# TencentARC/SEED-Story

Hardware: AMD Instinct MI355X
Metric: story-steps/sec (text + 1024x1024 image) (higher is better)
Workload: dtype bf16

## Files before the change

seed-story_amd/csrc/ss_attn.hip:

```cpp
#include "ss_common.h"

namespace ss {

struct AttnArgs {
    const void *q, *k, *v;
    void* out;
    int q_len, kv_len, hd, n_heads;
    int64_t q_sb, q_sh, q_ss, k_sb, k_sh, k_ss, v_sb, v_sh, v_ss, o_sb, o_sh, o_ss;
    float scale;
    int causal_br;
    int xcd_heads;
    int ragged;
    int kv_len_b[8];
};

template <typename T> struct AttnMma;
template <> struct AttnMma<bf16_t> {
    static __device__ __forceinline__ f32x4_t run(const uint4& a, const uint4& b, f32x4_t c) {
        return __builtin_amdgcn_mfma_f32_16x16x32_bf16(__builtin_bit_cast(bf16x8_t, a),
                                                       __builtin_bit_cast(bf16x8_t, b), c, 0, 0, 0);
    }
};
template <> struct AttnMma<f16_t> {
    static __device__ __forceinline__ f32x4_t run(const uint4& a, const uint4& b, f32x4_t c) {
// ... 896 lines not shown

#if SS_EXPERIMENTAL
template <typename T>
__global__ __launch_bounds__(256) __attribute__((amdgpu_waves_per_eu(2)))
void cross_attn64_kernel(const AttnArgs a, int n_items, int items_per_block, int chunks_per_pair) {
    constexpr int HD = 64, NDB = 4, NKB = 4, NKS = 2;
    const int tid = threadIdx.x, lane = tid & 63;
    const int wid = __builtin_amdgcn_readfirstlane(tid >> 6);
    const int l15 = lane & 15, grp = lane >> 4;
    const float sl2 = a.scale * 1.4426950408889634f;
    const uint4 ones = make_uint4(OnesFrag<T>::kPair, OnesFrag<T>::kPair, OnesFrag<T>::kPair, OnesFrag<T>::kPair);
    const int kvl = a.kv_len;
    const bool o_vec = ((a.o_ss | a.o_sh | a.o_sb) & 3) == 0;
    int it = blockIdx.x * items_per_block;
    int it_end = it + items_per_block;
    if (it_end > n_items) it_end = n_items;
    if (it >= it_end) return;

    uint4 kf[NKB][NKS];
    uint4 vf[NKB / 2][NDB];
    int cur_pair = -1;
    auto load_q = [&](int item, uint4 (&qf)[2][NKS]) {
        const int pair = item / chunks_per_pair, chunk = item - pair * chunks_per_pair;
        const int b = pair / a.n_heads, h = pair - b * a.n_heads;
        const T* __restrict__ qp = (const T*)a.q + (int64_t)b * a.q_sb + (int64_t)h * a.q_sh;
#pragma unroll
        for (int qb = 0; qb < 2; ++qb) {
            const int qi = chunk * 128 + wid * 32 + qb * 16 + l15;
#pragma unroll
            for (int ks = 0; ks < NKS; ++ks)
                qf[qb][ks] = qi < a.q_len ? ld16(qp + (int64_t)qi * a.q_ss + ks * 32 + grp * 8) : make_uint4(0, 0, 0, 0);
        }
    };
    uint4 qf[2][NKS], qn[2][NKS];
    load_q(it, qf);
    for (; it < it_end; ++it) {
        const bool more = it + 1 < it_end;
        if (more) load_q(it + 1, qn);
        const int pair = it / chunks_per_pair, chunk = it - pair * chunks_per_pair;
        const int b = pair / a.n_heads, h = pair - b * a.n_heads;
        if (pair != cur_pair) {
            cur_pair = pair;
            const T* __restrict__ kp = (const T*)a.k + (int64_t)b * a.k_sb + (int64_t)h * a.k_sh;
            const T* __restrict__ vp = (const T*)a.v + (int64_t)b * a.v_sb + (int64_t)h * a.v_sh;
#pragma unroll
            for (int kb = 0; kb < NKB; ++kb) {
                const int key = kb * 16 + l15;
#pragma unroll
                for (int ks = 0; ks < NKS; ++ks)
                    kf[kb][ks] = key < kvl ? ld16(kp + (int64_t)key * a.k_ss + ks * 32 + grp * 8) : make_uint4(0, 0, 0, 0);
            }
#pragma unroll
            for (int kp2 = 0; kp2 < NKB / 2; ++kp2)
#pragma unroll
                for (int db = 0; db < NDB; ++db) {
                    uint32_t w[4];
#pragma unroll
                    for (int j = 0; j < 8; j += 2) {
                        const int k0 = (2 * kp2 + (j >> 2)) * 16 + grp * 4 + (j & 3), k1 = k0 + 1;
                        const uint32_t lo = k0 < kvl ? (uint32_t)(vp + (int64_t)k0 * a.v_ss + db * 16 + l15)->v : 0u;
                        const uint32_t hi = k1 < kvl ? (uint32_t)(vp + (int64_t)k1 * a.v_ss + db * 16 + l15)->v : 0u;
                        w[j >> 1] = lo | (hi << 16);
                    }
                    vf[kp2][db] = make_uint4(w[0], w[1], w[2], w[3]);
                }
        }
        f32x4_t s[2][NKB];
#pragma unroll
        for (int kb = 0; kb < NKB; ++kb) {
            s[0][kb] = f32x4_t{0.f, 0.f, 0.f, 0.f};
            s[1][kb] = f32x4_t{0.f, 0.f, 0.f, 0.f};
#pragma unroll
            for (int ks = 0; ks < NKS; ++ks) {
                s[0][kb] = AttnMma<T>::run(kf[kb][ks], qf[0][ks], s[0][kb]);
                s[1][kb] = AttnMma<T>::run(kf[kb][ks], qf[1][ks], s[1][kb]);
            }
        }
        uint4 pfrag[2][NKB / 2];
#pragma unroll
        for (int qb = 0; qb < 2; ++qb) {
            if (kvl < 64) {
#pragma unroll
                for (int kb = 0; kb < NKB; ++kb)
#pragma unroll
                    for (int r = 0; r < 4; ++r)
                        if (kb * 16 + grp * 4 + r >= kvl) s[qb][kb][r] = -1e30f;
            }
            float tmax = -1e30f;
#pragma unroll
            for (int kb = 0; kb < NKB; ++kb)
#pragma unroll
                for (int r = 0; r < 4; ++r) tmax = fmaxf(tmax, s[qb][kb][r]);
            tmax = fmaxf(tmax, __shfl_xor(tmax, 16, 64));
            tmax = fmaxf(tmax, __shfl_xor(tmax, 32, 64));
            const float nm = -fmaxf(tmax, -1e29f) * sl2;
#pragma unroll
            for (int kp2 = 0; kp2 < NKB / 2; ++kp2) {
                float pf[8];
#pragma unroll
                for (int r = 0; r < 4; ++r) {
                    pf[r] = __builtin_amdgcn_exp2f(fmaf(s[qb][2 * kp2][r], sl2, nm));
                    pf[4 + r] = __builtin_amdgcn_exp2f(fmaf(s[qb][2 * kp2 + 1][r], sl2, nm));
                }
                pfrag[qb][kp2] = pack<T>(pf);
            }
        }
        f32x4_t o[2][NDB], osum[2];
#pragma unroll
        for (int qb = 0; qb < 2; ++qb) {
            osum[qb] = f32x4_t{0.f, 0.f, 0.f, 0.f};
#pragma unroll
            for (int i = 0; i < NDB; ++i) o[qb][i] = f32x4_t{0.f, 0.f, 0.f, 0.f};
        }
#pragma unroll
        for (int kp2 = 0; kp2 < NKB / 2; ++kp2) {
            osum[0] = AttnMma<T>::run(ones, pfrag[0][kp2], osum[0]);
            osum[1] = AttnMma<T>::run(ones, pfrag[1][kp2], osum[1]);
#pragma unroll
            for (int db = 0; db < NDB; ++db) {
                o[0][db] = AttnMma<T>::run(vf[kp2][db], pfrag[0][kp2], o[0][db]);
                o[1][db] = AttnMma<T>::run(vf[kp2][db], pfrag[1][kp2], o[1][db]);
            }
        }
#pragma unroll
        for (int qb = 0; qb < 2; ++qb) {
            const int qi = chunk * 128 + wid * 32 + qb * 16 + l15;
            if (qi >= a.q_len) continue;
            const float l = osum[qb][0];
            const float inv = l > 0.f ? 1.0f / l : 0.f;
            T* op = (T*)a.out + (int64_t)b * a.o_sb + (int64_t)h * a.o_sh + (int64_t)qi * a.o_ss;
#pragma unroll
            for (int db = 0; db < NDB; ++db) {
                const int d = db * 16 + grp * 4;
                if (o_vec) {
                    float pk[8] = {o[qb][db][0] * inv, o[qb][db][1] * inv, o[qb][db][2] * inv, o[qb][db][3] * inv, 0, 0, 0, 0};
                    const uint4 u = pack<T>(pk);
                    *reinterpret_cast<uint2*>(op + d) = make_uint2(u.x, u.y);
                } else {
#pragma unroll
                    for (int r = 0; r < 4; ++r) Tr<T>::st(op + d + r, o[qb][db][r] * inv);
                }
            }
        }
        if (more) {
#pragma unroll
            for (int qb = 0; qb < 2; ++qb)
#pragma unroll
                for (int ks = 0; ks < NKS; ++ks) qf[qb][ks] = qn[qb][ks];
        }
    }
}

template <typename T>
static int cross_attn64_launch(const AttnArgs& a, int64_t batch, hipStream_t s) {
    const int cpp = cdiv(a.q_len, 128);
    const int64_t n_items = batch * a.n_heads * cpp;
    static int n_cu = 0;
    if (n_cu == 0) {
        int dev = 0;
        hipDeviceProp_t p;
        if (hipGetDevice(&dev) == hipSuccess && hipGetDeviceProperties(&p, dev) == hipSuccess) n_cu = p.multiProcessorCount;
        if (n_cu <= 0) n_cu = 256;
    }
    const int64_t max_blocks = (int64_t)2 * n_cu;
    const int ipb = (int)((n_items + max_blocks - 1) / max_blocks);
    const int grid = (int)((n_items + ipb - 1) / ipb);
    hipLaunchKernelGGL((cross_attn64_kernel<T>), dim3((unsigned)grid), dim3(256), 0, s, a, (int)n_items, ipb, cpp);
    SS_LAUNCH_CHECK("cross_attn64");
    return SS_OK;
}

#endif

template <typename T, bool PIPE>
static int flash3p_launch(const AttnArgs& a, int64_t batch, hipStream_t s) {
    const int64_t kv_tiles = a.ragged ? 3 : cdiv(a.kv_len, kBKV);
    const size_t lds = (size_t)(kv_tiles < 3 && !PIPE ? (kv_tiles < 1 ? 1 : kv_tiles) : 3) * 2 * kBKV * 64 * 2;
    const int64_t bh = batch * a.n_heads;
    const int aw = knob(K_attn_waves);
    const bool many = a.ragged || a.kv_len >= 512;
    const bool w16 = !PIPE && (aw == 16 || (aw == 0 && many && a.q_len >= 2048 && (int64_t)cdiv(a.q_len, 512) * bh >= 1024));
    const bool w8 = !PIPE && !w16 && (aw == 8 || (aw == 0 && many && a.q_len >= 512 && (int64_t)cdiv(a.q_len, 256) * bh >= 1024));
    const int nqb = cdiv(a.q_len, w16 ? 512 : w8 ? 256 : 128);
    AttnArgs a2 = a;
    dim3 grid((unsigned)nqb, (unsigned)bh);
    a2.xcd_heads = 0;
    if (bh % 8 == 0 && nqb > 1 && knob(K_attn_xcd)) {
        a2.xcd_heads = nqb;
        grid = dim3((unsigned)(nqb * bh), 1);
    }
    if constexpr (!PIPE) {
        if (w16) {
            hipLaunchKernelGGL((flash_attn3p_kernel<T, 64, false, 16>), grid, dim3(1024), lds, s, a2);
            SS_LAUNCH_CHECK("flash_attn3p");
            return SS_OK;
        }
        if (w8) {
            hipLaunchKernelGGL((flash_attn3p_kernel<T, 64, false, 8>), grid, dim3(512), lds, s, a2);
            SS_LAUNCH_CHECK("flash_attn3p");
            return SS_OK;
        }
    }
    hipLaunchKernelGGL((flash_attn3p_kernel<T, 64, PIPE>), grid, dim3(256), lds, s, a2);
    SS_LAUNCH_CHECK("flash_attn3p");
    return SS_OK;
}

template <typename T, int HD, bool VSWZ>
static int flash3_launch_hd(const AttnArgs& a, int64_t batch, hipStream_t s) {
    const size_t lds = (size_t)(HD <= 64 ? 3 : 2) * 2 * kBKV * HD * 2;
    const int nqb = cdiv(a.q_len, 128);
    const int64_t bh = batch * a.n_heads;
    AttnArgs a2 = a;
    dim3 grid((unsigned)nqb, (unsigned)bh);
    a2.xcd_heads = 0;
    if (bh % 8 == 0 && nqb > 1 && knob(K_attn_xcd)) {
        a2.xcd_heads = nqb;
        grid = dim3((unsigned)(nqb * bh), 1);
    }
    hipLaunchKernelGGL((flash_attn3_kernel<T, HD, VSWZ>), grid, dim3(256), lds, s, a2);
    SS_LAUNCH_CHECK("flash_attn3");
    return SS_OK;
}

#if SS_EXPERIMENTAL
template <typename T, int HD>
static int flash2_launch_hd(const AttnArgs& a, int64_t batch, hipStream_t s) {
    const size_t lds = (size_t)(HD <= 64 ? 3 : 2) * 2 * kBKV * HD * 2;
    dim3 grid((unsigned)cdiv(a.q_len, 128), (unsigned)(batch * a.n_heads));
    hipLaunchKernelGGL((flash_attn2_kernel<T, HD>), grid, dim3(256), lds, s, a);
    SS_LAUNCH_CHECK("flash_attn2");
    return SS_OK;
}
#endif

template <typename T, int HD>
static int flash_launch_hd(const AttnArgs& a, int64_t batch, hipStream_t s) {
    constexpr int V = Tr<T>::kVec;
    const size_t lds = ((size_t)kBKV * (HD + V) + (size_t)HD * (kBKV + V)) * sizeof(T);
    dim3 grid((unsigned)cdiv(a.q_len, kBQ), (unsigned)(batch * a.n_heads));
    hipLaunchKernelGGL((flash_attn_kernel<T, HD>), grid, dim3(256), lds, s, a);
    SS_LAUNCH_CHECK("flash_attn");
    return SS_OK;
}

template <typename T>
int attention_launch(const AttnArgs& a, int64_t batch, hipStream_t s) {
    constexpr int V = Tr<T>::kVec;
    SS_REQUIRE(a.hd % V == 0 && a.hd > 0 && a.hd <= 128, "attention: head_dim %d unsupported", a.hd);
    SS_REQUIRE(a.q_ss % V == 0 && a.k_ss % V == 0 && a.v_ss % V == 0 && a.q_sh % V == 0 && a.k_sh % V == 0 &&
                   a.v_sh % V == 0 && a.q_sb % V == 0 && a.k_sb % V == 0 && a.v_sb % V == 0,
               "attention: strides must be multiples of %d elements", V);
    SS_REQUIRE(!a.causal_br || a.kv_len >= a.q_len, "attention: causal needs kv_len >= q_len");
    if (a.q_len == 0 || batch == 0) return SS_OK;
    SS_REQUIRE(a.kv_len > 0, "attention: kv_len == 0");
    if constexpr (V == 8) {
        const int ver = knob(K_attn_ver);
#if SS_EXPERIMENTAL
        if (a.hd == 64 && a.kv_len <= 64 && !a.causal_br && !a.ragged && a.q_len >= 128 && ver >= 3 && knob(K_attn_cross64))
            return cross_attn64_launch<T>(a, batch, s);
#endif
        if (ver == 5 && a.q_len >= 32 && a.hd <= 64) return flash3p_launch<T, true>(a, batch, s);
        if (ver == 6 && a.q_len >= 32 && a.hd <= 64) return flash3p_launch<T, false>(a, batch, s);
        if (ver >= 3 && a.q_len >= 32) {
            if (ver == 3 || ver >= 5) {
                if (a.hd <= 64) return flash3_launch_hd<T, 64, true>(a, batch, s);
                return flash3_launch_hd<T, 128, true>(a, batch, s);
            }
            if (a.hd <= 64) return flash3_launch_hd<T, 64, false>(a, batch, s);
            return flash3_launch_hd<T, 128, false>(a, batch, s);
        }
#if SS_EXPERIMENTAL
        if (ver == 2 && a.q_len >= 32) {
            if (a.hd <= 64) return flash2_launch_hd<T, 64>(a, batch, s);
            return flash2_launch_hd<T, 128>(a, batch, s);
        }
#else
        SS_REQUIRE(ver != 2, "attention: attn_ver 2 (flash v2) is only in the EXPERIMENTAL=1 build");
#endif
    }
    if (a.hd <= 64) return flash_launch_hd<T, 64>(a, batch, s);
    return flash_launch_hd<T, 128>(a, batch, s);
}

int attention_dev(const AttnArgs& a, int64_t batch, int dtype, hipStream_t s) {
    return SS_DISPATCH(dtype, attention_launch, a, batch, s);
}

template <typename T>
__device__ __forceinline__ uint4 rope_pack(const T* row_h, const T* cos_t, const T* sin_t, int pos, int hd, int d0) {
    constexpr int V = Tr<T>::kVec;
    const int half = hd >> 1;
    float x[V], xp[V], c[V], sn[V], o[V];
    unpack<T>(ld16(row_h + d0), x);
    unpack<T>(ld16(row_h + (d0 < half ? d0 + half : d0 - half)), xp);
    unpack<T>(ld16(cos_t + (int64_t)pos * hd + d0), c);
    unpack<T>(ld16(sin_t + (int64_t)pos * hd + d0), sn);
    const float sign = d0 < half ? -1.f : 1.f;
#pragma unroll
    for (int j = 0; j < V; ++j) o[j] = Tr<T>::rnd(Tr<T>::rnd(x[j] * c[j]) + Tr<T>::rnd(sign * xp[j] * sn[j]));
    return pack<T>(o);
}

struct DecodeArgs {
    const void* q;
    const void* qkv_raw;
    void *kc, *vc;
    const void *cos_t, *sin_t;
    float* part;
    const int32_t* kv_len_dev;
    const int32_t* pos_dev;
    const int32_t* done_flag;
    int hd, n_heads, cap, nsplit;
    float scale;
    int nb, state_stride;
    int64_t q_stride, cache_stride, part_stride, out_stride;
};

template <typename T>
__global__ __launch_bounds__(256) void attn_decode_kernel(const DecodeArgs a0) {
    DecodeArgs a = a0;
    {
        const int b = blockIdx.z;
        const int64_t so = (int64_t)b * a.state_stride;
        if (a.done_flag) a.done_flag += so;
        a.kv_len_dev += so;
        if (a.pos_dev) a.pos_dev += so;
        if (a.q) a.q = (const T*)a.q + b * a.q_stride;
        if (a.qkv_raw) a.qkv_raw = (const T*)a.qkv_raw + b * a.q_stride;
        a.kc = (T*)a.kc + b * a.cache_stride;
        a.vc = (T*)a.vc + b * a.cache_stride;
        a.part += b * a.part_stride;
    }
    constexpr int V = Tr<T>::kVec;
    constexpr int KPT = 4;
    extern __shared__ __attribute__((aligned(16))) char smem_raw[];
    float* sm = reinterpret_cast<float*>(smem_raw);
    if (a.done_flag && *a.done_flag) return;
    const int h = blockIdx.x, sp = blockIdx.y, tid = threadIdx.x;
    const int hd = a.hd;
    const int LPK = hd / V, NKG = 256 / LPK;
    const int kg = tid / LPK, dl = tid % LPK, d0 = dl * V;
    const bool fused = a.qkv_raw != nullptr;
    const int n_old = *a.kv_len_dev;
    const int kv_len = n_old + (fused ? 1 : 0);
    const int chunk = (kv_len + a.nsplit - 1) / a.nsplit;
    const int k_lo = sp * chunk;
    const int k_hi = min(kv_len, k_lo + chunk);
    const T* kh = (const T*)a.kc + (int64_t)h * a.cap * hd;
    const T* vh = (const T*)a.vc + (int64_t)h * a.cap * hd;
    const int E = a.n_heads * hd;

    auto load_kv = [&](int base, uint4 (&kk)[KPT], uint4 (&vv)[KPT]) {
#pragma unroll
        for (int i = 0; i < KPT; ++i) {
            const int key = base + i * NKG;
            if (key < k_hi && !(fused && key == n_old)) {
                kk[i] = ld16(kh + (int64_t)key * hd + d0);
                vv[i] = ld16(vh + (int64_t)key * hd + d0);
            } else {
                kk[i] = make_uint4(0, 0, 0, 0);
                vv[i] = make_uint4(0, 0, 0, 0);
            }
        }
    };
    uint4 kk[KPT], vv[KPT];
    int base = k_lo + kg;
    if (base < k_hi) load_kv(base, kk, vv);

    uint4 qv, knew = make_uint4(0, 0, 0, 0), vnew = make_uint4(0, 0, 0, 0);
    if (fused) {
        const T* raw = (const T*)a.qkv_raw;
        const int pos = *a.pos_dev;
        qv = rope_pack<T>(raw + (int64_t)h * hd, (const T*)a.cos_t, (const T*)a.sin_t, pos, hd, d0);
        if (n_old >= k_lo && n_old < k_hi) {
            knew = rope_pack<T>(raw + E + (int64_t)h * hd, (const T*)a.cos_t, (const T*)a.sin_t, pos, hd, d0);
            vnew = ld16(raw + 2 * E + (int64_t)h * hd + d0);
            if (kg == (n_old - k_lo) % NKG && n_old < a.cap) {
                st16((T*)a.kc + ((int64_t)h * a.cap + n_old) * hd + d0, knew);
                st16((T*)a.vc + ((int64_t)h * a.cap + n_old) * hd + d0, vnew);
            }
        }
    } else {
        qv = ld16((const T*)a.q + (int64_t)h * hd + d0);
    }

    float m = -1e30f, l = 0.f, acc[V];
#pragma unroll
    for (int j = 0; j < V; ++j) acc[j] = 0.f;
    while (base < k_hi) {
#pragma unroll
        for (int i = 0; i < KPT; ++i) {
            const int key = base + i * NKG;
            const bool is_new = fused && key == n_old;
            const uint4 kx = is_new ? knew : kk[i];
            const uint4 vx = is_new ? vnew : vv[i];
            float s = dot_pack<T>(kx, qv, 0.f);
            for (int o = LPK >> 1; o > 0; o >>= 1) s += __shfl_xor(s, o, 64);
            if (key < k_hi) {
                s *= a.scale;
                const float mn = fmaxf(m, s);
                const float al = expf(m - mn), p = expf(s - mn);
                float vf[V];
                unpack<T>(vx, vf);
                l = l * al + p;
#pragma unroll
                for (int j = 0; j < V; ++j) acc[j] = fmaf(p, vf[j], acc[j] * al);
                m = mn;
            }
        }
        base += NKG * KPT;
        if (base < k_hi) load_kv(base, kk, vv);
    }
    float* mine = sm + kg * (hd + 2);
    if (dl == 0) { mine[0] = m; mine[1] = l; }
#pragma unroll
    for (int j = 0; j < V; ++j) mine[2 + d0 + j] = acc[j];
    __syncthreads();
    float* rec = a.part + ((int64_t)h * a.nsplit + sp) * (hd + 2);
    if (tid < hd) {
        float mm = -1e30f;
        for (int g = 0; g < NKG; ++g) mm = fmaxf(mm, sm[g * (hd + 2)]);
        float lt = 0.f, ot = 0.f;
        for (int g = 0; g < NKG; ++g) {
            const float* r = sm + g * (hd + 2);
            const float w = r[1] > 0.f ? expf(r[0] - mm) : 0.f;
            lt = fmaf(w, r[1], lt);
            ot = fmaf(w, r[2 + tid], ot);
        }
        rec[2 + tid] = ot;
        if (tid == 0) { rec[0] = mm; rec[1] = lt; }
    }
}

template <typename T, int NS>
__global__ void attn_combine_kernel(const float* __restrict__ part, T* __restrict__ out,
                                    const int32_t* __restrict__ done_flag, int hd, int state_stride,
                                    int64_t part_stride, int64_t out_stride) {
    const int b = blockIdx.y;
    if (done_flag && done_flag[(int64_t)b * state_stride]) return;
    part += b * part_stride;
    out += b * out_stride;
    const int h = blockIdx.x, d = threadIdx.x;
    const float* rec = part + (int64_t)h * NS * (hd + 2);
    float ms[NS], ls[NS], os[NS];
#pragma unroll
    for (int s = 0; s < NS; ++s) {
        ms[s] = rec[s * (hd + 2)];
        ls[s] = rec[s * (hd + 2) + 1];
        os[s] = rec[s * (hd + 2) + 2 + d];
    }
    float m = -1e30f;
#pragma unroll
    for (int s = 0; s < NS; ++s) m = fmaxf(m, ms[s]);
    float l = 0.f, o = 0.f;
#pragma unroll
    for (int s = 0; s < NS; ++s) {
        const float w = ls[s] > 0.f ? expf(ms[s] - m) : 0.f;
        l = fmaf(w, ls[s], l);
        o = fmaf(w, os[s], o);
    }
    Tr<T>::st(out + (int64_t)h * hd + d, o / l);
}

static inline int decode_nsplit(int nb) {
    int n = knob(K_attn_decode_nsplit);
    if (n <= 0) n = 16 / (nb < 1 ? 1 : nb);
    return n <= 4 ? 4 : n <= 8 ? 8 : n <= 16 ? 16 : 32;
}

template <typename T>
int attn_decode_launch(const DecodeArgs& a0, void* out, int64_t n_heads, int64_t hd, hipStream_t s) {
    constexpr int V = Tr<T>::kVec;
    SS_REQUIRE(hd % V == 0 && 256 % (hd / V) == 0 && 64 % (hd / V) == 0 && hd <= 256,
               "attn_decode: head_dim %lld unsupported", (long long)hd);
    DecodeArgs a = a0;
    a.nsplit = decode_nsplit(a.nb);
    a.scale = 1.0f / sqrtf((float)hd);
    const int NKG = 256 / (int)(hd / V);
    const size_t lds = (size_t)NKG * (hd + 2) * sizeof(float);
    if (a.nb < 1) a.nb = 1;
    hipLaunchKernelGGL(attn_decode_kernel<T>, dim3((unsigned)n_heads, (unsigned)a.nsplit, (unsigned)a.nb), dim3(256),
                       lds, s, a);
    SS_LAUNCH_CHECK("attn_decode");
#define SS_COMBINE(NS)                                                                                          \
    hipLaunchKernelGGL((attn_combine_kernel<T, NS>), dim3((unsigned)n_heads, (unsigned)a.nb), dim3((unsigned)hd), 0, \
                       s, (const float*)a.part, (T*)out, a.done_flag, (int)hd, a.state_stride, a.part_stride,       \
                       a.out_stride)
    switch (a.nsplit) {
        case 4: SS_COMBINE(4); break;
        case 8: SS_COMBINE(8); break;
        case 16: SS_COMBINE(16); break;
        default: SS_COMBINE(32); break;
    }
#undef SS_COMBINE
    SS_LAUNCH_CHECK("attn_combine");
    return SS_OK;
}

int attn_decode_dev(const void* q, const void* kc, const void* vc, void* out, void* ws, const int32_t* kv_len_dev,
                    const int32_t* done_flag, int64_t n_heads, int64_t hd, int64_t cache_cap, int dtype,
                    hipStream_t s) {
    DecodeArgs a;
    a.q = q; a.qkv_raw = nullptr; a.kc = (void*)kc; a.vc = (void*)vc; a.cos_t = a.sin_t = nullptr;
    a.part = (float*)ws; a.kv_len_dev = kv_len_dev; a.pos_dev = nullptr; a.done_flag = done_flag;
    a.hd = (int)hd; a.n_heads = (int)n_heads; a.cap = (int)cache_cap; a.nsplit = 0; a.scale = 0.f;
    a.nb = 1; a.state_stride = 0; a.q_stride = a.cache_stride = a.part_stride = a.out_stride = 0;
    return SS_DISPATCH(dtype, attn_decode_launch, a, out, n_heads, hd, s);
}

int attn_decode_fused_dev(const void* qkv_raw, void* kc, void* vc, const void* cos_t, const void* sin_t, void* out,
                          void* ws, const int32_t* kv_len_dev, const int32_t* pos_dev, const int32_t* done_flag,
                          int64_t n_heads, int64_t hd, int64_t cache_cap, int nb, int state_stride,
                          int64_t cache_stride, int dtype, hipStream_t s) {
    DecodeArgs a;
    a.nb = nb; a.state_stride = state_stride; a.q_stride = 3 * n_heads * hd; a.cache_stride = cache_stride;
    a.part_stride = (int64_t)(ss_attn_decode_workspace_bytes(n_heads, hd) / sizeof(float));
    a.out_stride = n_heads * hd;
    a.q = nullptr; a.qkv_raw = qkv_raw; a.kc = kc; a.vc = vc; a.cos_t = cos_t; a.sin_t = sin_t;
    a.part = (float*)ws; a.kv_len_dev = kv_len_dev; a.pos_dev = pos_dev; a.done_flag = done_flag;
    a.hd = (int)hd; a.n_heads = (int)n_heads; a.cap = (int)cache_cap; a.nsplit = 0; a.scale = 0.f;
    return SS_DISPATCH(dtype, attn_decode_launch, a, out, n_heads, hd, s);
}

}

using namespace ss;

extern "C" {

int ss_attention(const void* q, const void* k, const void* v, void* out, int64_t batch, int64_t n_heads,
                 int64_t q_len, int64_t kv_len, int64_t hd, int64_t q_sb, int64_t q_sh, int64_t q_ss, int64_t k_sb,
                 int64_t k_sh, int64_t k_ss, int64_t v_sb, int64_t v_sh, int64_t v_ss, int64_t o_sb, int64_t o_sh,
                 int64_t o_ss, float scale, int causal_br, int dtype, void* stream) {
    AttnArgs a;
    a.q = q; a.k = k; a.v = v; a.out = out;
    a.q_len = (int)q_len; a.kv_len = (int)kv_len; a.hd = (int)hd; a.n_heads = (int)n_heads;
    a.q_sb = q_sb; a.q_sh = q_sh; a.q_ss = q_ss; a.k_sb = k_sb; a.k_sh = k_sh; a.k_ss = k_ss;
    a.v_sb = v_sb; a.v_sh = v_sh; a.v_ss = v_ss; a.o_sb = o_sb; a.o_sh = o_sh; a.o_ss = o_ss;
    a.scale = scale; a.causal_br = causal_br; a.xcd_heads = 0; a.ragged = 0;
    return attention_dev(a, batch, dtype, (hipStream_t)stream);
}

int ss_attention_ragged(const void* q, const void* k, const void* v, void* out, int64_t batch, int64_t n_heads, int64_t q_len,
                        const int32_t* host_kv_lens, int64_t hd, int64_t q_sb, int64_t q_sh, int64_t q_ss, int64_t k_sb,
                        int64_t k_sh, int64_t k_ss, int64_t v_sb, int64_t v_sh, int64_t v_ss, int64_t o_sb, int64_t o_sh,
                        int64_t o_ss, float scale, int causal_br, int dtype, void* stream) {
    SS_REQUIRE(host_kv_lens && batch >= 1 && batch <= 8, "attention_ragged: 1..8 batch elements");
    AttnArgs a;
    a.q = q; a.k = k; a.v = v; a.out = out;
    a.q_len = (int)q_len; a.hd = (int)hd; a.n_heads = (int)n_heads;
    a.q_sb = q_sb; a.q_sh = q_sh; a.q_ss = q_ss; a.k_sb = k_sb; a.k_sh = k_sh; a.k_ss = k_ss;
    a.v_sb = v_sb; a.v_sh = v_sh; a.v_ss = v_ss; a.o_sb = o_sb; a.o_sh = o_sh; a.o_ss = o_ss;
    a.scale = scale; a.causal_br = causal_br; a.xcd_heads = 0; a.ragged = 1;
    int mx = 0;
    for (int b = 0; b < 8; ++b) {
        a.kv_len_b[b] = b < batch ? host_kv_lens[b] : 0;
        if (b < batch) {
            SS_REQUIRE(host_kv_lens[b] > 0 && (!causal_br || host_kv_lens[b] >= q_len), "attention_ragged: kv_len[%d] = %d", b,
                       (int)host_kv_lens[b]);
            if (host_kv_lens[b] > mx) mx = host_kv_lens[b];
        }
    }
    a.kv_len = mx;
    return attention_dev(a, batch, dtype, (hipStream_t)stream);
}

size_t ss_attn_decode_workspace_bytes(int64_t n_heads, int64_t hd) {
    return (size_t)n_heads * 64  * (size_t)(hd + 2) * sizeof(float);
}

int ss_attn_decode(const void* q, const void* kcache, const void* vcache, void* out, void* workspace,
                   const int32_t* kv_len_dev, int64_t n_heads, int64_t hd, int64_t cache_cap, int dtype,
                   void* stream) {
    return attn_decode_dev(q, kcache, vcache, out, workspace, kv_len_dev, nullptr, n_heads, hd, cache_cap, dtype,
                           (hipStream_t)stream);
}

}
```

Before: 2.334.

## Fuse split-KV combine into decode attention via atomic last-block ticket

Removes the separate combine kernel. Each split block bumps a per-head atomic ticket, and the last block to arrive merges all partial records and writes the bf16 output. The inner loop now takes a block of KPT keys at a time: one max, one rescale, exp2 with a pre-scaled log2 factor, and branch-free clamped K/V prefetch loads. This cuts one launch per decode step and some transcendental work, but relies on the tickets starting at zero (memset only on the non-fused path) and adds fences/atomics on the tail.

```diff
diff --git a/seed-story_amd/csrc/ss_attn.hip b/seed-story_amd/csrc/ss_attn.hip
--- a/seed-story_amd/csrc/ss_attn.hip
+++ b/seed-story_amd/csrc/ss_attn.hip
@@ -1222,12 +1222,17 @@
     return pack<T>(o);
 }
 
+__device__ __forceinline__ uint4 sel16(bool c, const uint4& a, const uint4& b) {
+    return make_uint4(c ? a.x : b.x, c ? a.y : b.y, c ? a.z : b.z, c ? a.w : b.w);
+}
+
 struct DecodeArgs {
     const void* q;
     const void* qkv_raw;
     void *kc, *vc;
     const void *cos_t, *sin_t;
     float* part;
+    void* out;
     const int32_t* kv_len_dev;
     const int32_t* pos_dev;
     const int32_t* done_flag;
@@ -1236,6 +1241,9 @@
     int nb, state_stride;
     int64_t q_stride, cache_stride, part_stride, out_stride;
 };
+
+constexpr int kDecodeMaxSplit = 64;
+static inline size_t decode_ticket_bytes(int64_t n_heads) { return ((size_t)n_heads * sizeof(unsigned) + 15) / 16 * 16; }
 
 template <typename T>
 __global__ __launch_bounds__(256) void attn_decode_kernel(const DecodeArgs a0) {
@@ -1251,6 +1259,7 @@
         a.kc = (T*)a.kc + b * a.cache_stride;
         a.vc = (T*)a.vc + b * a.cache_stride;
         a.part += b * a.part_stride;
+        a.out = (T*)a.out + b * a.out_stride;
     }
     constexpr int V = Tr<T>::kVec;
     constexpr int KPT = 4;
@@ -1271,22 +1280,16 @@
     const T* vh = (const T*)a.vc + (int64_t)h * a.cap * hd;
     const int E = a.n_heads * hd;
 
-    auto load_kv = [&](int base, uint4 (&kk)[KPT], uint4 (&vv)[KPT]) {
-#pragma unroll
-        for (int i = 0; i < KPT; ++i) {
-            const int key = base + i * NKG;
-            if (key < k_hi && !(fused && key == n_old)) {
-                kk[i] = ld16(kh + (int64_t)key * hd + d0);
-                vv[i] = ld16(vh + (int64_t)key * hd + d0);
-            } else {
-                kk[i] = make_uint4(0, 0, 0, 0);
-                vv[i] = make_uint4(0, 0, 0, 0);
-            }
-        }
+    const int step = NKG * KPT;
+    const int n_iter = k_hi > k_lo ? (k_hi - k_lo + step - 1) / step : 0;
+    const int last_row = min(k_hi, a.cap) - 1;
+    auto load_rows = [&](const T* plane, int base, uint4 (&r)[KPT]) {
+#pragma unroll
+        for (int i = 0; i < KPT; ++i) r[i] = ld16(plane + (int64_t)min(base + i * NKG, last_row) * hd + d0);
     };
     uint4 kk[KPT], vv[KPT];
     int base = k_lo + kg;
-    if (base < k_hi) load_kv(base, kk, vv);
+    if (n_iter > 0) { load_rows(kh, base, kk); load_rows(vh, base, vv); }
 
     uint4 qv, knew = make_uint4(0, 0, 0, 0), vnew = make_uint4(0, 0, 0, 0);
     if (fused) {
@@ -1305,33 +1308,48 @@
         qv = ld16((const T*)a.q + (int64_t)h * hd + d0);
     }
 
+    const float sl2 = a.scale * 1.4426950408889634f;
     float m = -1e30f, l = 0.f, acc[V];
 #pragma unroll
     for (int j = 0; j < V; ++j) acc[j] = 0.f;
-    while (base < k_hi) {
+    auto sub_chunk = [&](auto prefetch) {
+        float s[KPT];
 #pragma unroll
         for (int i = 0; i < KPT; ++i) {
-            const int key = base + i * NKG;
-            const bool is_new = fused && key == n_old;
-            const uint4 kx = is_new ? knew : kk[i];
-            const uint4 vx = is_new ? vnew : vv[i];
-            float s = dot_pack<T>(kx, qv, 0.f);
-            for (int o = LPK >> 1; o > 0; o >>= 1) s += __shfl_xor(s, o, 64);
-            if (key < k_hi) {
-                s *= a.scale;
-                const float mn = fmaxf(m, s);
-                const float al = expf(m - mn), p = expf(s - mn);
-                float vf[V];
-                unpack<T>(vx, vf);
-                l = l * al + p;
-#pragma unroll
-                for (int j = 0; j < V; ++j) acc[j] = fmaf(p, vf[j], acc[j] * al);
-                m = mn;
-            }
-        }
-        base += NKG * KPT;
-        if (base < k_hi) load_kv(base, kk, vv);
-    }
+            const uint4 kx = sel16(fused && base + i * NKG == n_old, knew, kk[i]);
+            s[i] = dot_pack<T>(kx, qv, 0.f);
+        }
+        if (prefetch) load_rows(kh, base + step, kk);
+        for (int o = LPK >> 1; o > 0; o >>= 1) {
+#pragma unroll
+            for (int i = 0; i < KPT; ++i) s[i] += __shfl_xor(s[i], o, 64);
+        }
+        float mn = m;
+#pragma unroll
+        for (int i = 0; i < KPT; ++i) {
+            s[i] = base + i * NKG < k_hi ? s[i] * sl2 : -1e30f;
+            mn = fmaxf(mn, s[i]);
+        }
+        const float al = __builtin_amdgcn_exp2f(m - mn);
+        l *= al;
+#pragma unroll
+        for (int j = 0; j < V; ++j) acc[j] *= al;
+#pragma unroll
+        for (int i = 0; i < KPT; ++i) {
+            const float p = base + i * NKG < k_hi ? __builtin_amdgcn_exp2f(s[i] - mn) : 0.f;
+            const uint4 vx = sel16(fused && base + i * NKG == n_old, vnew, vv[i]);
+            float vf[V];
+            unpack<T>(vx, vf);
+            l += p;
+#pragma unroll
+            for (int j = 0; j < V; ++j) acc[j] = fmaf(p, vf[j], acc[j]);
+        }
+        if (prefetch) load_rows(vh, base + step, vv);
+        m = mn;
+        base += step;
+    };
+    for (int it = 1; it < n_iter; ++it) sub_chunk(std::true_type{});
+    if (n_iter > 0) sub_chunk(std::false_type{});
     float* mine = sm + kg * (hd + 2);
     if (dl == 0) { mine[0] = m; mine[1] = l; }
 #pragma unroll
@@ -1344,43 +1362,45 @@
         float lt = 0.f, ot = 0.f;
         for (int g = 0; g < NKG; ++g) {
             const float* r = sm + g * (hd + 2);
-            const float w = r[1] > 0.f ? expf(r[0] - mm) : 0.f;
+            const float w = r[1] > 0.f ? __builtin_amdgcn_exp2f(r[0] - mm) : 0.f;
             lt = fmaf(w, r[1], lt);
             ot = fmaf(w, r[2 + tid], ot);
         }
         rec[2 + tid] = ot;
         if (tid == 0) { rec[0] = mm; rec[1] = lt; }
     }
-}
-
-template <typename T, int NS>
-__global__ void attn_combine_kernel(const float* __restrict__ part, T* __restrict__ out,
-                                    const int32_t* __restrict__ done_flag, int hd, int state_stride,
-                                    int64_t part_stride, int64_t out_stride) {
-    const int b = blockIdx.y;
-    if (done_flag && done_flag[(int64_t)b * state_stride]) return;
-    part += b * part_stride;
-    out += b * out_stride;
-    const int h = blockIdx.x, d = threadIdx.x;
-    const float* rec = part + (int64_t)h * NS * (hd + 2);
-    float ms[NS], ls[NS], os[NS];
-#pragma unroll
-    for (int s = 0; s < NS; ++s) {
-        ms[s] = rec[s * (hd + 2)];
-        ls[s] = rec[s * (hd + 2) + 1];
-        os[s] = rec[s * (hd + 2) + 2 + d];
-    }
-    float m = -1e30f;
-#pragma unroll
-    for (int s = 0; s < NS; ++s) m = fmaxf(m, ms[s]);
-    float l = 0.f, o = 0.f;
-#pragma unroll
-    for (int s = 0; s < NS; ++s) {
-        const float w = ls[s] > 0.f ? expf(ms[s] - m) : 0.f;
-        l = fmaf(w, ls[s], l);
-        o = fmaf(w, os[s], o);
-    }
-    Tr<T>::st(out + (int64_t)h * hd + d, o / l);
+    asm volatile("s_waitcnt vmcnt(0)" ::: "memory");
+    __syncthreads();
+    int* is_last = reinterpret_cast<int*>(sm + NKG * (hd + 2));
+    if (tid == 0) {
+        unsigned* ticket = reinterpret_cast<unsigned*>(a.part + (int64_t)a.n_heads * kDecodeMaxSplit * (hd + 2)) + h;
+        __builtin_amdgcn_fence(__ATOMIC_RELEASE, "agent");
+        asm volatile("s_waitcnt vmcnt(0)" ::: "memory");
+        const unsigned t = __hip_atomic_fetch_add(ticket, 1u, __ATOMIC_RELAXED, __HIP_MEMORY_SCOPE_AGENT);
+        const bool last = t == (unsigned)a.nsplit - 1u;
+        if (last) {
+            __builtin_amdgcn_fence(__ATOMIC_ACQUIRE, "agent");
+            asm volatile("s_waitcnt vmcnt(0)" ::: "memory");
+            __hip_atomic_store(ticket, 0u, __ATOMIC_RELAXED, __HIP_MEMORY_SCOPE_AGENT);
+        }
+        *is_last = last;
+    }
+    __syncthreads();
+    if (!*is_last || tid >= hd) return;
+    const float* recs = a.part + (int64_t)h * a.nsplit * (hd + 2);
+    auto ldrec = [&](int i) { return __hip_atomic_load(recs + i, __ATOMIC_RELAXED, __HIP_MEMORY_SCOPE_AGENT); };
+    float mm = -1e30f;
+#pragma unroll 4
+    for (int s = 0; s < a.nsplit; ++s) mm = fmaxf(mm, ldrec(s * (hd + 2)));
+    float lt = 0.f, ot = 0.f;
+#pragma unroll 4
+    for (int s = 0; s < a.nsplit; ++s) {
+        const float ms = ldrec(s * (hd + 2)), ls = ldrec(s * (hd + 2) + 1), os = ldrec(s * (hd + 2) + 2 + tid);
+        const float w = ls > 0.f ? __builtin_amdgcn_exp2f(ms - mm) : 0.f;
+        lt = fmaf(w, ls, lt);
+        ot = fmaf(w, os, ot);
+    }
+    Tr<T>::st((T*)a.out + (int64_t)h * hd + tid, ot / lt);
 }
 
 static inline int decode_nsplit(int nb) {
@@ -1390,7 +1410,7 @@
 }
 
 template <typename T>
-int attn_decode_launch(const DecodeArgs& a0, void* out, int64_t n_heads, int64_t hd, hipStream_t s) {
+int attn_decode_launch(const DecodeArgs& a0, int64_t n_heads, int64_t hd, hipStream_t s) {
     constexpr int V = Tr<T>::kVec;
     SS_REQUIRE(hd % V == 0 && 256 % (hd / V) == 0 && 64 % (hd / V) == 0 && hd <= 256,
                "attn_decode: head_dim %lld unsupported", (long long)hd);
@@ -1398,23 +1418,11 @@
     a.nsplit = decode_nsplit(a.nb);
     a.scale = 1.0f / sqrtf((float)hd);
     const int NKG = 256 / (int)(hd / V);
-    const size_t lds = (size_t)NKG * (hd + 2) * sizeof(float);
+    const size_t lds = ((size_t)NKG * (hd + 2) * sizeof(float) + 15) / 16 * 16 + 16;
     if (a.nb < 1) a.nb = 1;
     hipLaunchKernelGGL(attn_decode_kernel<T>, dim3((unsigned)n_heads, (unsigned)a.nsplit, (unsigned)a.nb), dim3(256),
                        lds, s, a);
     SS_LAUNCH_CHECK("attn_decode");
-#define SS_COMBINE(NS)                                                                                          \
-    hipLaunchKernelGGL((attn_combine_kernel<T, NS>), dim3((unsigned)n_heads, (unsigned)a.nb), dim3((unsigned)hd), 0, \
-                       s, (const float*)a.part, (T*)out, a.done_flag, (int)hd, a.state_stride, a.part_stride,       \
-                       a.out_stride)
-    switch (a.nsplit) {
-        case 4: SS_COMBINE(4); break;
-        case 8: SS_COMBINE(8); break;
-        case 16: SS_COMBINE(16); break;
-        default: SS_COMBINE(32); break;
-    }
-#undef SS_COMBINE
-    SS_LAUNCH_CHECK("attn_combine");
     return SS_OK;
 }
 
@@ -1423,10 +1431,12 @@
                     hipStream_t s) {
     DecodeArgs a;
     a.q = q; a.qkv_raw = nullptr; a.kc = (void*)kc; a.vc = (void*)vc; a.cos_t = a.sin_t = nullptr;
-    a.part = (float*)ws; a.kv_len_dev = kv_len_dev; a.pos_dev = nullptr; a.done_flag = done_flag;
+    a.part = (float*)ws; a.out = out; a.kv_len_dev = kv_len_dev; a.pos_dev = nullptr; a.done_flag = done_flag;
     a.hd = (int)hd; a.n_heads = (int)n_heads; a.cap = (int)cache_cap; a.nsplit = 0; a.scale = 0.f;
     a.nb = 1; a.state_stride = 0; a.q_stride = a.cache_stride = a.part_stride = a.out_stride = 0;
-    return SS_DISPATCH(dtype, attn_decode_launch, a, out, n_heads, hd, s);
+    const size_t rec_bytes = (size_t)n_heads * kDecodeMaxSplit * (size_t)(hd + 2) * sizeof(float);
+    SS_HIP(hipMemsetAsync((char*)ws + rec_bytes, 0, decode_ticket_bytes(n_heads), s));
+    return SS_DISPATCH(dtype, attn_decode_launch, a, n_heads, hd, s);
 }
 
 int attn_decode_fused_dev(const void* qkv_raw, void* kc, void* vc, const void* cos_t, const void* sin_t, void* out,
@@ -1438,9 +1448,9 @@
     a.part_stride = (int64_t)(ss_attn_decode_workspace_bytes(n_heads, hd) / sizeof(float));
     a.out_stride = n_heads * hd;
     a.q = nullptr; a.qkv_raw = qkv_raw; a.kc = kc; a.vc = vc; a.cos_t = cos_t; a.sin_t = sin_t;
-    a.part = (float*)ws; a.kv_len_dev = kv_len_dev; a.pos_dev = pos_dev; a.done_flag = done_flag;
+    a.part = (float*)ws; a.out = out; a.kv_len_dev = kv_len_dev; a.pos_dev = pos_dev; a.done_flag = done_flag;
     a.hd = (int)hd; a.n_heads = (int)n_heads; a.cap = (int)cache_cap; a.nsplit = 0; a.scale = 0.f;
-    return SS_DISPATCH(dtype, attn_decode_launch, a, out, n_heads, hd, s);
+    return SS_DISPATCH(dtype, attn_decode_launch, a, n_heads, hd, s);
 }
 
 }
@@ -1487,7 +1497,7 @@
 }
 
 size_t ss_attn_decode_workspace_bytes(int64_t n_heads, int64_t hd) {
-    return (size_t)n_heads * 64  * (size_t)(hd + 2) * sizeof(float);
+    return (size_t)n_heads * kDecodeMaxSplit * (size_t)(hd + 2) * sizeof(float) + decode_ticket_bytes(n_heads);
 }
 
 int ss_attn_decode(const void* q, const void* kcache, const void* vcache, void* out, void* workspace,
```

New measurement: 2.316. About the same (-0.8%).
